# MaciejKozarzewski/AlphaGomoku

Hardware: AMD Instinct MI355X
Metric: MCTS simulations/sec (self-play, 15x15 freestyle) (higher is better)
Workload: dtype f16 (network, fp32 accumulate) + int/fp32 (tree)

## Files before the change

alphagomoku_amd/_lib.py:

```python
import ctypes
import os

_HERE = os.path.dirname(os.path.abspath(__file__))
LIB_PATH = os.environ.get("AGX_LIB_PATH") or os.path.join(_HERE, "libagx.so")


class AgxError(RuntimeError):
    pass


class AgxNetDesc(ctypes.Structure):
    _fields_ = [("rows", ctypes.c_int), ("cols", ctypes.c_int), ("blocks", ctypes.c_int),
                ("filters", ctypes.c_int), ("in_channels", ctypes.c_int), ("value_hidden", ctypes.c_int),
                ("action_values", ctypes.c_int)]


_shared_torch_runtime = None


def share_torch_hip_runtime():
    global _shared_torch_runtime
    if _shared_torch_runtime is not None:
        return _shared_torch_runtime
    import importlib.util
# ... 88 lines not shown
def check(status):
    if status != 0:
        raise AgxError("agx error %d: %s" % (status, lib.agx_last_error().decode()))


class AgxEngineConfig(ctypes.Structure):
    _fields_ = [("rules", ctypes.c_int), ("board_size", ctypes.c_int), ("draw_after", ctypes.c_int), ("n_games", ctypes.c_int),
                ("max_batch_size", ctypes.c_int), ("max_simulations", ctypes.c_int), ("exploration_constant", ctypes.c_float),
                ("exploration_scaling", ctypes.c_float), ("init_to", ctypes.c_int), ("information_leak_threshold", ctypes.c_float),
                ("policy_expansion_threshold", ctypes.c_float), ("tss_max_positions", ctypes.c_int),
                ("tss_table_entries", ctypes.c_uint64), ("zobrist_seed", ctypes.c_uint64), ("node_capacity", ctypes.c_int),
                ("edge_capacity", ctypes.c_int), ("record_capacity", ctypes.c_int), ("record_edge_capacity", ctypes.c_int),
                ("solver_yield_fraction", ctypes.c_float), ("final_selector", ctypes.c_int), ("use_symmetries", ctypes.c_int),
                ("symmetry_seed", ctypes.c_uint64), ("max_children", ctypes.c_int), ("noise_type", ctypes.c_int), ("noise_weight", ctypes.c_float),
                ("noise_seed", ctypes.c_uint64), ("action_values", ctypes.c_int), ("match_mode", ctypes.c_int), ("policy_temperature", ctypes.c_float),
                ("arena_reserve", ctypes.c_float), ("search_threads", ctypes.c_int), ("record_format", ctypes.c_int), ("record_sample_capacity", ctypes.c_int), ("game_end_capacity", ctypes.c_int),
                ("speculative_solver", ctypes.c_int), ("speculative_waves", ctypes.c_int), ("force_expand_root", ctypes.c_int), ("search_buffers", ctypes.c_int)]


class AgxEngineBuffers(ctypes.Structure):
    _fields_ = [("d_nn_features", ctypes.c_void_p), ("d_nn_policy", ctypes.c_void_p), ("d_nn_value", ctypes.c_void_p),
                ("d_nn_action_values", ctypes.c_void_p),
                ("d_nn_list", ctypes.c_void_p), ("d_nn_count", ctypes.c_void_p), ("slots", ctypes.c_int), ("cells", ctypes.c_int)]


class AgxEngineStats(ctypes.Structure):
    _fields_ = [(n, ctypes.c_ulonglong) for n in
                ["evaluated_nodes", "network_evaluations", "information_leaks", "proven_edge_visits", "wasted_expansions",
                 "duplicate_selections", "solver_nodes", "select_levels", "select_edge_reads", "moves_played", "peak_nodes",
                 "peak_edges"]] + [(n, ctypes.c_int) for n in
                                   ["games_finished", "openings_taken", "active_games", "records_used", "record_edges_used",
                                    "first_error", "arena_grows", "arena_releases", "arena_failures", "arena_max_class"]] + \
               [("arena_heap_used", ctypes.c_float), ("speculative_parks", ctypes.c_int), ("speculative_solves", ctypes.c_ulonglong),
                ("speculative_reruns", ctypes.c_ulonglong), ("speculative_deferrals", ctypes.c_ulonglong)]


class AgxEdgeView(ctypes.Structure):
    _fields_ = [("prior", ctypes.c_float), ("win", ctypes.c_float), ("draw", ctypes.c_float), ("visits", ctypes.c_int32),
                ("move", ctypes.c_uint16), ("score", ctypes.c_uint16), ("flag_and_virtual_loss", ctypes.c_uint16),
                ("reserved", ctypes.c_uint16)]


class AgxNodeView(ctypes.Structure):
    _fields_ = [("found", ctypes.c_int), ("visits", ctypes.c_int), ("win", ctypes.c_float), ("draw", ctypes.c_float), ("moves_left", ctypes.c_float)] + \
               [(n, ctypes.c_int) for n in ["score", "flags", "sign_to_move", "depth", "virtual_loss", "n_edges"]]


class AgxGameInfo(ctypes.Structure):
    _fields_ = [(n, ctypes.c_int) for n in ["active", "sign_to_move", "n_moves", "outcome", "error", "opening_id", "games_done",
                                            "n_nodes", "n_edges", "root_visits"]] + \
               [("root_win", ctypes.c_float), ("root_draw", ctypes.c_float), ("root_score", ctypes.c_int), ("root_edges", ctypes.c_int),
                ("grow_pending", ctypes.c_int), ("arena_class", ctypes.c_int), ("root_moves_left", ctypes.c_float), ("max_depth", ctypes.c_int)]


class AgxMoveRecord(ctypes.Structure):
    _fields_ = [("game_serial", ctypes.c_int), ("move_number", ctypes.c_int), ("move", ctypes.c_uint16), ("root_score", ctypes.c_uint16),
                ("root_visits", ctypes.c_int), ("root_win", ctypes.c_float), ("root_draw", ctypes.c_float), ("n_edges", ctypes.c_int),
                ("edge_offset", ctypes.c_int), ("root_flags", ctypes.c_int), ("game_slot", ctypes.c_int), ("game_index", ctypes.c_int),
                ("sample_offset", ctypes.c_int), ("sample_bytes", ctypes.c_int), ("outcome", ctypes.c_int)]


class AgxGameEnd(ctypes.Structure):
    _fields_ = [("game_serial", ctypes.c_int), ("game_slot", ctypes.c_int), ("game_index", ctypes.c_int), ("outcome", ctypes.c_int),
                ("n_moves", ctypes.c_int), ("moves", ctypes.c_uint16 * 400)]


class AgxSavedGame(ctypes.Structure):
# ... 146 lines not shown
```

alphagomoku_amd/csrc/dev_solver.hpp:

```cpp
#ifndef AGX_DEV_SOLVER_HPP_
#define AGX_DEV_SOLVER_HPP_

#include <hip/hip_runtime.h>
#include "engine_types.hpp"

namespace agx
{
	namespace dev
	{
		typedef uint64_t u64;

		__device__ __forceinline__ void wave_sync()
		{
			__builtin_amdgcn_wave_barrier();
			__builtin_amdgcn_fence(__ATOMIC_ACQ_REL, "wavefront");
			__builtin_amdgcn_wave_barrier();
		}

#define AGX_DPP_STEP(V, OP, CTRL, ROWS) V = OP(V, static_cast<uint32_t>(__builtin_amdgcn_update_dpp(0, static_cast<int>(V), CTRL, ROWS, 0xf, false)))
#define AGX_OP_MAX(a, b) max(a, b)
#define AGX_OP_ADD(a, b) ((a) + (b))
#define AGX_OP_XOR(a, b) ((a) ^ (b))
#define AGX_OP_OR(a, b) ((a) | (b))
#define AGX_WAVE_REDUCE(V, OP) do { AGX_DPP_STEP(V, OP, 0x111, 0xf); AGX_DPP_STEP(V, OP, 0x112, 0xf); AGX_DPP_STEP(V, OP, 0x114, 0xf); \
// ... 108 lines not shown
		{
			win = 0.0f;
			draw = 0.0f;
			switch (s_pv(d))
			{
				case 1: draw = 1.0f; break;
				case 2: win = (1000 + s_eval(d)) / 2000.0f; break;
				case 3: win = s_infinite(d) ? 0.0f : 1.0f; break;
				default: break;
			}
		}

		struct alignas(16) Frame
		{
				int base;
				uint16_t size, i;
				uint16_t alpha, beta, original_alpha, best_score;
				uint16_t best_move, move, baseline;
				int16_t depth_remaining;
				uint8_t must_defend, has_initiative, fully_expanded, pad;
				uint32_t ov_slot;
		};
		static_assert(sizeof(Frame) == 32, "frame layout");
		enum Cmd : int { CMD_NONE = 0, CMD_ADD = 1, CMD_UNDO = 2, CMD_DONE = 3 };
#ifndef AGX_LUT_LDS
#define AGX_LUT_LDS 0
#endif
#ifndef AGX_PLACE_OPAQUE_LANE
#define AGX_PLACE_OPAQUE_LANE 1
#endif
		constexpr int NODE_TIME_OVER = 0x40000000;
		constexpr int NODE_COUNT_MASK = NODE_TIME_OVER - 1;
		constexpr int LDS_FRAMES = 42;
		constexpr int OV_CAP = 256;

		template<int N>
		struct SolverSharedT
		{
				static constexpr int DIM = N, HW = N * N;
				static constexpr int CAP2 = (N <= 15) ? 64 : 96, CAP = 24;
				static constexpr int LIST_ITEMS = CAP2 + 7 * CAP;
				static constexpr int SELECT_KEY_BYTES = 3 * (1 + HW) * 8;
#ifndef AGX_ACT_LDS_20
#define AGX_ACT_LDS_20 336
#endif
				static constexpr int ACT_LDS = (N <= 15) ? 448 : AGX_ACT_LDS_20;
				static constexpr int FRAMES = (N <= 15) ? 30 : 34;
				__device__ static constexpr int list_cap(int t) { return (t == 2) ? CAP2 : CAP; }
				__device__ static constexpr int list_off(int t) { return (t == 2) ? 0 : CAP2 + (t - 3) * CAP; }

				u64 lines[6 * N];
				uint32_t act[ACT_LDS];
				Frame frames[FRAMES];
				uint8_t ptype[HW][8];
#if AGX_LUT_LDS
				uint8_t threat_lut[4096];
#endif
				uint8_t threat[HW][2];
				uint16_t items[2][LIST_ITEMS];
				uint16_t pos[2][HW];
				alignas(4) uint16_t count[2][10];
				uint32_t legal[N];
				uint32_t added[N];
				uint32_t row_mask[N];
				uint16_t tmp_list[HW];
				uint16_t foul_cell[64];
				uint8_t foul_flag[64];
				uint8_t board[(HW + 7) / 8 * 8];
				int foul_count;
				int fstack[16][5];
				u64 pf_bucket[8];
				u64 pf_lo;
				int pf_valid;
				uint32_t ov_keys[OV_CAP];
				uint32_t ov_dirty[OV_CAP / 32];
				u64 *ov_data;
				int ov_on, ov_count, ov_overflow, pf_slot;
#ifdef AGX_SOLVER_PROFILE
				unsigned long long prof[8];
				unsigned long long dprof[24];
#endif
				alignas(16) u64 hash_lo;
				u64 hash_hi;
				int phase, level, node_counter, stack_offset;
				int stack_max, error, pending_value, cmd_move;
				u64 time_deadline;
				uint16_t *spill_lists;
				alignas(16) u64 *snap;
				int sign_to_move, depth;
				Frame *spill_frames;
				int cmd, result_score;
		};
		typedef SolverSharedT<MAXN> SolverShared;
#if !defined(AGX_SOLVER_PROFILE)
		static_assert(sizeof(SolverSharedT<15>) <= 10240, "15x15 solver state: sixteen waves per compute unit (160 KB of LDS)");
#endif

		template<class SH>
		__device__ __forceinline__ uint32_t list_get(const SH &sh, int s, int t, int i)
		{
			if (__builtin_expect(i < SH::list_cap(t), 1))
				return sh.items[s][SH::list_off(t) + i];
			uint32_t v;
			asm volatile("global_load_ushort %0, %1, off\n\ts_waitcnt vmcnt(0)" : "=v"(v) : "v"(sh.spill_lists + (s * 10 + t) * SH::HW + i) : "memory");
			return v;
		}
		template<class SH>
		__device__ __forceinline__ void list_set(SH &sh, int s, int t, int i, uint32_t cell)
		{
			if (__builtin_expect(i < SH::list_cap(t), 1))
// ... 1584 lines not shown
						if (distance_to_draw >= 3)
							add_list(opp, 4, s_unknown(4), false);
						mark_neighborhood();
						create_remaining_moves(sh.row_mask, s_unknown(0));
					}
					AGX_PROF_MARK(sh, 7);
					if (fouls_possible_for(own))
						mark_forbidden_moves();
					AGX_PROF_MARK(sh, 9);
					f.fully_expanded = (f.must_defend || mode >= 2) ? 1 : 0;
					return result;
				}
		};

		template<class SH>
		__device__ __forceinline__ int ov_find(const SH &sh, uint32_t bucket, int lane)
		{
			const int cnt = sh.ov_count;
			lane = fresh_lane(lane);
			for (int base = 0; base < cnt; base += 64)
			{
				const u64 m = __ballot(base + lane < cnt && sh.ov_keys[base + lane] == bucket);
				if (m != 0)
					return base + __ffsll(static_cast<long long>(m)) - 1;
			}
			return -1;
		}
		template<class SH>
		__device__ __forceinline__ int ov_create(SH &sh, uint32_t bucket, u64 word, int lane)
		{
			const int p = sh.ov_count;
			if (p >= OV_CAP)
			{
				sh.ov_overflow = 1;
				return -1;
			}
			if (lane < 16)
				global_view(sh.ov_data)[p * 16 + lane] = word;
			if (lane == 0)
			{
				sh.ov_keys[p] = bucket;
				sh.ov_count = p + 1;
			}
			wave_sync();
			return p;
		}

		__device__ __forceinline__ u64 tt_pack(int bound, int depth, uint32_t score, uint32_t move)
		{
			return static_cast<u64>(bound) | (static_cast<u64>(depth) << 8) | (static_cast<u64>(score) << 16) | (static_cast<u64>(move) << 32);
		}
		__device__ __forceinline__ u64 tt_seek(const u64 *tt, u64 bucket_mask, u64 lo, u64 hi)
		{
			const u64 *bucket = tt + 8 * (lo & bucket_mask);
			const u64 KEY = 0xFFFF000000000000ull;
			for (int i = 0; i < 4; i++)
				if (bucket[2 * i] == hi && (bucket[2 * i + 1] & KEY) == (lo & KEY))
					return bucket[2 * i + 1];
			return tt_pack(0, 0, s_unknown(0), 0);
		}
		__device__ __forceinline__ void tt_insert(u64 *tt, u64 bucket_mask, u64 lo, u64 hi, u64 value, int generation)
		{
			const u64 KEY = 0xFFFF000000000000ull;
			value &= ~(KEY | 0xFCull);
			value |= static_cast<u64>(generation) << 2;
			value |= (lo & KEY);
			u64 *bucket = tt + 8 * (lo & bucket_mask);
			const uint32_t score = static_cast<uint32_t>((value >> 16) & 65535u);
			if (s_proven(score) || (value & 3ull) == 3ull)
				for (int i = 0; i < 4; i++)
					if (bucket[2 * i] == hi && (bucket[2 * i + 1] & KEY) == (lo & KEY))
					{
						bucket[2 * i] = hi;
						bucket[2 * i + 1] = value;
						return;
					}
			int idx = 0, best_worth = 0;
			for (int i = 0; i < 4; i++)
// ... 3 lines not shown
				if (i == 0 || worth < best_worth)
				{
					best_worth = worth;
					idx = i;
				}
			}
			bucket[2 * idx] = hi;
			bucket[2 * idx + 1] = value;
		}

#ifndef AGX_TT_LANES
#define AGX_TT_LANES 1
#endif
		__device__ __forceinline__ u64 wave_read64(u64 v, int src_lane)
		{
			const int l = __builtin_amdgcn_readfirstlane(src_lane);
			const uint32_t lo = static_cast<uint32_t>(__builtin_amdgcn_readlane(static_cast<int>(static_cast<uint32_t>(v)), l));
			const uint32_t hi = static_cast<uint32_t>(__builtin_amdgcn_readlane(static_cast<int>(static_cast<uint32_t>(v >> 32)), l));
			return static_cast<u64>(lo) | (static_cast<u64>(hi) << 32);
		}
		__device__ __forceinline__ int tt_match_lanes(u64 word, u64 lo, u64 hi, int lane)
		{
			const u64 KEY = 0xFFFF000000000000ull;
			const bool mine = (lane < 8) && (((lane & 1) == 0) ? (word == hi) : ((word & KEY) == (lo & KEY)));
			const uint32_t m = static_cast<uint32_t>(__ballot(mine));
			const uint32_t both = m & (m >> 1) & 0x55u;
			return (both != 0u) ? ((__ffs(static_cast<int>(both)) - 1) >> 1) : -1;
		}
		__device__ __forceinline__ u64 tt_seek_lanes(u64 word, u64 lo, u64 hi, int lane)
		{
			const int k = tt_match_lanes(word, lo, hi, lane);
			return (k >= 0) ? wave_read64(word, 2 * k + 1) : tt_pack(0, 0, s_unknown(0), 0);
		}
		__device__ __forceinline__ void tt_insert_lanes(u64 *bucket, u64 lo, u64 hi, u64 value, int generation, int lane)
		{
			const u64 KEY = 0xFFFF000000000000ull;
			value &= ~(KEY | 0xFCull);
			value |= static_cast<u64>(generation) << 2;
			value |= (lo & KEY);
			u64 word = 0;
			if (lane < 8)
				word = global_view(bucket)[lane];
			const uint32_t score = static_cast<uint32_t>((value >> 16) & 65535u);
			int idx = -1;
			if (s_proven(score) || (value & 3ull) == 3ull)
				idx = tt_match_lanes(word, lo, hi, lane);
			if (idx < 0)
			{
				const int worth = static_cast<int>((word >> 8) & 255) - (generation - static_cast<int>((word >> 2) & 63));
				const int w0 = __builtin_amdgcn_readlane(worth, 1), w1 = __builtin_amdgcn_readlane(worth, 3), w2 = __builtin_amdgcn_readlane(worth, 5),
						w3 = __builtin_amdgcn_readlane(worth, 7);
				idx = 0;
				int best = w0;
				if (w1 < best) { best = w1; idx = 1; }
				if (w2 < best) { best = w2; idx = 2; }
				if (w3 < best) { best = w3; idx = 3; }
			}
			if (lane < 2)
				global_view(bucket)[2 * idx + lane] = (lane == 0) ? hi : value;
		}

		template<class SH>
		__device__ __forceinline__ uint32_t solver_evaluate(const SH &sh)
		{
			const int lane = static_cast<int>(threadIdx.x);
			const int own = sh.sign_to_move - 1;
			int product = 0;
			if (lane < 20)
			{
				const int side = (lane >= 10) ? 1 : 0, t = lane - 10 * side;
				constexpr u64 OWN_WEIGHTS = 19ull | (49ull << 8) | (76ull << 16) | (170ull << 24) | (33ull << 32) | (159ull << 40) | (252ull << 48);
				constexpr u64 OPP_WEIGHTS = 1ull | (50ull << 9) | (45ull << 18) | (135ull << 27) | (14ull << 36) | (154ull << 45) | (496ull << 54);
				const bool mine = (side == own), weighs = (t >= 2 && t <= 8);
				const int field = weighs ? t - 2 : 0;
				const int magnitude = static_cast<int>(((mine ? OWN_WEIGHTS : OPP_WEIGHTS) >> ((mine ? 8 : 9) * field)) & (mine ? 255ull : 511ull));
				const int weight = weighs ? (mine ? magnitude : -magnitude) : 0;
				product = weight * static_cast<int>(sh.count[side][t]);
			}
			const int result = 12 + static_cast<int>(wave_reduce_add(static_cast<uint32_t>(product)));
			return s_unknown(max(-1000, min(1000, result)));
		}

		template<bool RENJU, class SH>
		__device__ __forceinline__ int solver_run(SH &sh, const EngineDev &E, uint32_t *act, u64 *tt, int generation, int lane, u64 &pf_word,
				uint8_t &pf_pattern, int &pf_pattern_tag, u64 &pf_snap)
		{
			AGX_PROF_BEGIN();
			const u64 zseed = E.zobrist_seed;
			const int n = E.n;
			int phase = sh.phase, level = sh.level;
// ... 12 lines not shown
				sh.error = error;
				sh.hash_lo = hash_lo;
				sh.hash_hi = hash_hi;
				sh.pending_value = static_cast<int>(value);
				sh.cmd_move = move;
				return cmd;
			};
			uint32_t cur_action = 0;
			while (true)
			{
				bool returning = false;
				AGX_PROF_COUNT(sh, 21, 1);
#ifdef AGX_SOLVER_PROFILE
				agx_pt_ = clock64();
				const unsigned long long p0 = wall_clock64();
				unsigned long long p1 = p0, p2 = p0;
#endif
				if (phase == 0)
				{
					f.best_move = 0;
					u64 entry;
					const bool have_pf = sh.pf_valid && sh.pf_lo == hash_lo;
					if (have_pf || sh.ov_on)
					{
						if (sh.ov_on)
						{
							const uint32_t bucket = static_cast<uint32_t>(hash_lo & E.tt_bucket_mask);
							int slot = have_pf ? sh.pf_slot : ov_find(sh, bucket, lane);
							if (!have_pf && lane < 16)
								pf_word = (slot >= 0) ? global_view(sh.ov_data)[slot * 16 + 8 + (lane & 7)] : global_view(tt)[8 * static_cast<u64>(bucket) + (lane & 7)];
							if (slot < 0)
								slot = ov_create(sh, bucket, pf_word, lane);
							f.ov_slot = static_cast<uint32_t>(slot);
						}
#if AGX_TT_LANES
						entry = tt_seek_lanes(pf_word, hash_lo, hash_hi, lane);
					}
					else
					{
						u64 word = 0;
						if (lane < 8)
							word = tt[8 * (hash_lo & E.tt_bucket_mask) + lane];
						entry = tt_seek_lanes(word, hash_lo, hash_hi, lane);
					}
#else
						if (lane < 8)
							sh.pf_bucket[lane] = pf_word;
						wave_sync();
						const u64 KEY = 0xFFFF000000000000ull;
						entry = tt_pack(0, 0, s_unknown(0), 0);
						for (int k = 3; k >= 0; k--)
							if (sh.pf_bucket[2 * k] == hash_hi && (sh.pf_bucket[2 * k + 1] & KEY) == (hash_lo & KEY))
								entry = sh.pf_bucket[2 * k + 1];
					}
					else
						entry = tt_seek(tt, E.tt_bucket_mask, hash_lo, hash_hi);
#endif
					sh.pf_valid = 0;
					bool early = false;
					if (sh.ov_on && sh.ov_overflow)
					{
						error = ERR_OVERLAY;
						value = s_unknown(0);
						early = true;
					}
					else if ((entry & 3ull) != 0ull)
					{
						f.best_move = static_cast<uint16_t>((entry >> 32) & 65535u);
						if (level != 0)
						{
							const uint32_t tt_s = static_cast<uint32_t>((entry >> 16) & 65535u);
							const int b = static_cast<int>(entry & 3ull);
							if (s_proven(tt_s))
							{
								value = tt_s;
								early = true;
							}
							else if (static_cast<int>((entry >> 8) & 255) >= f.depth_remaining && (b == 3 || (b == 1 && tt_s >= f.beta) || (b == 2 && tt_s <= f.alpha)))
							{
								value = tt_s;
								early = true;
							}
						}
					}
#ifdef AGX_SOLVER_PROFILE
					p1 = wall_clock64();
					sh.prof[0] += p1 - p0;
#endif
					if (!early)
					{
						node_counter++;
						if (E.solve_time_ticks != 0ull && wall_clock64() >= sh.time_deadline)
							node_counter |= NODE_TIME_OVER;
// ... 181 lines not shown
						continue;
					}
				}
#ifdef AGX_SOLVER_PROFILE
				const unsigned long long p4 = wall_clock64();
				sh.prof[2] += p4 - p3;
#endif
				if (!returning && phase == 4)
				{
					uint32_t best = f.best_score;
					if (f.size == 0 || (s_loss(best) && !f.fully_expanded))
						best = solver_evaluate(sh);
					if (level > 0)
					{
						const uint32_t umv = frame_get(sh, level - 1).move;
#if AGX_SNAPSHOT_UNDO && AGX_SNAPSHOT_PREFETCH
						pf_snap = *global_view(snap_address<SH>(sh.snap, sh.depth - 1, lane));
						pf_pattern_tag = static_cast<int>(umv);
#elif !AGX_SNAPSHOT_UNDO
						pf_pattern = pattern_prefetch(sh, E, n, umv, false, lane);
						pf_pattern_tag = static_cast<int>(umv);
#endif
					}
					int bound;
					if (best <= f.original_alpha)
						bound = 2;
					else
						bound = (best >= f.beta) ? 1 : 3;
					if (sh.ov_on)
					{
						if (error != ERR_OVERLAY)
						{
							const int slot = static_cast<int>(f.ov_slot);
#if AGX_TT_LANES
							tt_insert_lanes(sh.ov_data + slot * 16 + 8, hash_lo, hash_hi, tt_pack(bound, f.depth_remaining, best, f.best_move), generation, lane);
#else
							tt_insert(sh.ov_data + slot * 16 + 8, 0ull, hash_lo, hash_hi, tt_pack(bound, f.depth_remaining, best, f.best_move), generation);
#endif
							if (lane == 0)
								sh.ov_dirty[slot >> 5] |= 1u << (slot & 31);
						}
					}
					else
#if AGX_TT_LANES
						tt_insert_lanes(tt + 8 * (hash_lo & E.tt_bucket_mask), hash_lo, hash_hi, tt_pack(bound, f.depth_remaining, best, f.best_move), generation, lane);
#else
						tt_insert(tt, E.tt_bucket_mask, hash_lo, hash_hi, tt_pack(bound, f.depth_remaining, best, f.best_move), generation);
#endif
					value = best;
					returning = true;
#ifdef AGX_SOLVER_PROFILE
					sh.prof[3] += wall_clock64() - p4;
#endif
				}
				if (returning)
				{
					if (level == 0)
					{
						sh.frames[0] = f;
						sh.result_score = static_cast<int>(value);
						return yield(CMD_DONE, 0);
					}
					stack_offset -= f.size;
					level--;
					phase = 1;
					return yield(CMD_UNDO, frame_get(sh, level).move);
// ... 8 lines not shown
```

alphagomoku_amd/csrc/engine.hip:

```cpp
#include "agx_internal.hpp"
#include "engine_types.hpp"
#include "dev_mcts.hpp"
#include "tables_host.hpp"
#include "renju_static.hpp"
#include "root_noise.hpp"
#include "sample_v201.hpp"

#include <vector>
#include <thread>
#include <chrono>
#include <mutex>
#include <cstring>
#include <algorithm>

using namespace agx;
using namespace agx::dev;

namespace
{
	__device__ __forceinline__ void select_batch(EngineDev &E, int tg, int g, int lane, uint8_t *sh_board, u64 *sh_cboard, const u64 *sh_keys)
	{
		GameState &gs = E.games[tg];
		GameState &ls = E.games[g];
		DNode *nodes = nodes_of(E, tg, gs.arena);
// ... 289 lines not shown
		u64 *tt = E.tt + static_cast<size_t>(g % E.tt_mod) * (E.tt_bucket_mask + 1ull) * 8ull;
		const int parked_in = (park != nullptr) ? __builtin_amdgcn_readfirstlane(E.park_slot[slot]) : 0;
		int depth_first = 0, stack_before_first = 0;
		if (parked_in != 0)
		{
			static_assert(sizeof(SH) % 8 == 0 && sizeof(SH) / 8 <= SPEC_PARK_WORDS - 8, "park buffer holds the solver's LDS state");
			const u64 *src = E.park_lds + static_cast<size_t>(parked_in - 1) * SPEC_PARK_WORDS;
			u64 *lds = reinterpret_cast<u64*>(&sh);
			for (int i = fresh_lane(lane); i < static_cast<int>(sizeof(SH) / 8); i += 64)
				lds[i] = global_view(src)[i];
			depth_first = static_cast<int>(src[SPEC_PARK_WORDS - 8]);
			stack_before_first = static_cast<int>(src[SPEC_PARK_WORDS - 7]);
			wave_sync();
			park_copy_tails(sh, E, E.park_area0 + parked_in - 1, area, lane);
			if (lane == 0)
			{
				park_point_tails_at(sh, E, area);
				sh.pf_valid = 0;
				E.park_slot[slot] = 0;
			}
			__threadfence();
			wave_sync();
			if (lane == 0)
				__hip_atomic_store(&E.park_owner[parked_in - 1], 0, __ATOMIC_RELEASE, __HIP_MEMORY_SCOPE_AGENT);
		}
		else
		{
		if (lane == 0)
		{
			park_point_tails_at(sh, E, area);
			sh.ov_on = (overlay != nullptr) ? 1 : 0;
			sh.ov_data = overlay;
			sh.ov_count = 0;
			sh.ov_overflow = 0;
			sh.pf_slot = -1;
		}
		if (lane < OV_CAP / 32)
			sh.ov_dirty[lane] = 0;
		}
#ifdef AGX_SOLVER_PROFILE
		unsigned long long c0 = wall_clock64(), c_run = 0, c_place = 0, n_place = 0;
		unsigned long long c1 = c0, t_forbidden = 0;
#endif
		if (parked_in == 0)
		{
		solver_set_board(sh, E, t.board, t.sign_to_move, lane);
		solver_encode_features(sh, E, E.nn_features + static_cast<size_t>(slot) * E.hw, lane);
		#ifdef AGX_SOLVER_PROFILE
		const unsigned long long c_enc = wall_clock64();
		#endif
		if (RENJU)
			solver_encode_forbidden(sh, E, E.nn_features + static_cast<size_t>(slot) * E.hw, lane);
		#ifdef AGX_SOLVER_PROFILE
		c1 = wall_clock64();
		t_forbidden = c1 - c_enc;
		#endif
		u64 lo = 0, hi = 0;
		for (int i = lane; i < E.hw; i += 64)
		{
			const int v = sh.board[i];
			if (v == 1 || v == 2)
			{
				lo ^= zobrist_word(E.zobrist_seed, 2 * (2 * i + v - 1));
				hi ^= zobrist_word(E.zobrist_seed, 2 * (2 * i + v - 1) + 1);
			}
		}
		lo = wave_reduce_xor64(lo);
// ... 301 lines not shown
			{
				gs.solve_pos = k;
				gs.solve_pending = 1;
				gs.stats[5] += solver_nodes;
			}
			return;
		}
		const unsigned long long scheduled = idle ? 0ull : schedule_to_nn(sh, E, g, gs, n_tasks, lane);
		if (lane == 0)
		{
			if (!idle)
			{
				gs.solve_pos = 0;
				gs.solve_pending = 0;
				gs.stats[5] += solver_nodes;
				gs.stats[1] += scheduled;
			}
			atomicAdd(&E.counters[E.yield_counter], 1);
		}
	}


	template<class SH>
	__device__ __forceinline__ void spec_flush(const SH &sh, SpecTask &h, int nodes, uint32_t flags0, float moves_left0, int lane)
	{
		const int cnt = sh.ov_count;
		for (int i = lane; i < cnt; i += 64)
			h.keys[i] = sh.ov_keys[i];
		if (lane < OV_CAP / 32)
			h.dirty[lane] = sh.ov_dirty[lane];
		if (lane == 0)
		{
			h.count = cnt;
			h.overflow = (sh.ov_overflow || sh.error == ERR_OVERLAY) ? 1 : 0;
			h.nodes = nodes;
			h.flags0 = flags0;
			h.moves_left0 = moves_left0;
			h.solved = 1;
		}
	}
#ifndef AGX_DEFER_ON_EMPTY_QUEUE
#define AGX_DEFER_ON_EMPTY_QUEUE 0
#endif
	struct SpecCommit
	{
		int game, k, first;
			bool table_changed;
			unsigned long long nodes, solved, reruns;
	};
	template<class SH>
	__device__ __forceinline__ int spec_commit_game(SH &sh, const EngineDev &E, SpecCommit &c, int lane, const int *c_done, int defer_threshold, const int *c_queue, int count)
	{
		const int g = c.game;
		GameState &gs = E.games[g];
		const int n_tasks = gs.n_tasks;
		u64 *tt = E.tt + static_cast<size_t>(g % E.tt_mod) * (E.tt_bucket_mask + 1ull) * 8ull;
		for (int k = c.k; k < n_tasks; k++)
		{
			const int slot = g * E.batch + k;
			SpecTask &h = E.spec_tasks[slot];
			if (h.solved == 0)
				continue;
			DTask &t = E.tasks[slot];
			const u64 *ov = E.spec_overlay + static_cast<size_t>(slot) * (SPEC_OV_CAP * 16);
			const int cnt = h.count;
			bool valid = (h.overflow == 0);
			{
				bool bad = (cnt < 0 || cnt > SPEC_OV_CAP);
				for (int i = lane; !bad && i < cnt; i += 64)
					bad = static_cast<u64>(h.keys[i]) > E.tt_bucket_mask;
				if (__ballot(bad) != 0ull)
				{
					if (lane == 0)
					{
						gs.error = ERR_SPEC_STATE;
						h.solved = 0;
					}
					continue;
				}
			}
			if (valid && c.table_changed)
			{
				bool mismatch = false;
				for (int base = 0; base < cnt; base += 8)
				{
					const int p = base + (lane >> 3), w = lane & 7;
					if (p < cnt)
						mismatch = mismatch || (ov[p * 16 + w] != tt[8 * static_cast<u64>(h.keys[p]) + w]);
				}
				valid = (__ballot(mismatch) == 0ull);
			}
			if (!valid)
			{
				int done = 0;
				if (lane == 0)
					done = __hip_atomic_load(c_done, __ATOMIC_RELAXED, __HIP_MEMORY_SCOPE_AGENT);
#if AGX_DEFER_ON_EMPTY_QUEUE
				int dry = 0;
				if (lane == 0 && defer_threshold != 0x7FFFFFFF)
					dry = (__hip_atomic_load(c_queue + 3, __ATOMIC_RELAXED, __HIP_MEMORY_SCOPE_AGENT) >= count
							&& __hip_atomic_load(c_queue + 1, __ATOMIC_RELAXED, __HIP_MEMORY_SCOPE_AGENT) >= __hip_atomic_load(c_queue + 2, __ATOMIC_RELAXED, __HIP_MEMORY_SCOPE_AGENT)) ? 1 : 0;
				const bool defer = (__builtin_amdgcn_readfirstlane(done) >= defer_threshold || __builtin_amdgcn_readfirstlane(dry) != 0) && k > c.first;
#else
				const bool defer = __builtin_amdgcn_readfirstlane(done) >= defer_threshold && k > c.first;
#endif
				for (int j = k; j < (defer ? n_tasks : k + 1); j++)
				{
					SpecTask &hj = E.spec_tasks[g * E.batch + j];
					if (hj.solved != 0 && lane == 0)
					{
						DTask &tj = E.tasks[g * E.batch + j];
						tj.flags = hj.flags0;
						tj.win = 0.0f;
						tj.draw = 0.0f;
						tj.moves_left = hj.moves_left0;
						hj.solved = 0;
					}
				}
				wave_sync();
				if (defer)
				{
					if (lane == 0)
					{
						gs.solve_pos = k;
						gs.solve_pending = 1;
						gs.stats[5] += c.nodes;
						gs.spec_stats[0] += c.solved;
						gs.spec_stats[1] += c.reruns;
						gs.spec_stats[2] += 1;
					}
					return -2;
				}
				c.solved++;
				c.reruns++;
				c.table_changed = true;
				c.k = k + 1;
				return k;
			}
			bool any = false;
			for (int base = 0; base < cnt; base += 8)
			{
				const int p = base + (lane >> 3), w = lane & 7;
				if (p < cnt && ((h.dirty[p >> 5] >> (p & 31)) & 1u))
				{
					tt[8 * static_cast<u64>(h.keys[p]) + w] = ov[p * 16 + 8 + w];
					any = true;
				}
			}
			c.table_changed = c.table_changed || (__ballot(any) != 0ull);
			c.nodes += static_cast<unsigned long long>(h.nodes);
			c.solved++;
			if (lane == 0)
				h.solved = 0;
			wave_sync();
		}
		const unsigned long long scheduled = schedule_to_nn(sh, E, g, gs, n_tasks, lane);
		if (lane == 0)
		{
			gs.solve_pos = 0;
			gs.solve_pending = 0;
			gs.stats[5] += c.nodes;
			gs.stats[1] += scheduled;
			gs.spec_stats[0] += c.solved;
			gs.spec_stats[1] += c.reruns;
#ifdef AGX_SPEC_PROFILE
			E.spec_trace[4 * g + 3] = c.reruns * 16 + c.solved;
#endif
		}
		return -1;
	}

#ifdef AGX_SPEC_PROFILE
#define SPEC_T(var) unsigned long long var = wall_clock64()
#define SPEC_ADD(k, v) do { if (lane == 0) atomicAdd(&E.spec_prof[k], static_cast<unsigned long long>(v)); } while (0)
#define SPEC_MAX(k, v) do { if (lane == 0) atomicMax(&E.spec_prof[k], static_cast<unsigned long long>(v)); } while (0)
#define SPEC_WAVE_EXIT() do { if (lane == 0) { unsigned long long *w_ = E.spec_trace + 4 * (static_cast<size_t>(E.n_games) + E.spec_group * E.spec_waves + blockIdx.x); \
		w_[0] = t_selected; w_[1] = wall_clock64(); w_[2] = wave_solves; w_[3] = wave_waited; } } while (0)
#else
#define SPEC_T(var) do { } while (0)
#define SPEC_ADD(k, v) do { } while (0)
#define SPEC_MAX(k, v) do { } while (0)
#define SPEC_WAVE_EXIT() do { } while (0)
#endif
#ifndef AGX_SPEC_WAVES
#define AGX_SPEC_WAVES 3
#endif
#ifndef AGX_SPEC_WAVES_15
#define AGX_SPEC_WAVES_15 4
#endif
	constexpr int spec_waves_per_simd(int nfix) { return (nfix == 15) ? AGX_SPEC_WAVES_15 : AGX_SPEC_WAVES; }
	template<bool RENJU, int NFIX>
	__global__ __launch_bounds__(64, spec_waves_per_simd(NFIX)) void k_search_spec(EngineDev E, int count)
	{
		if (NFIX != 0)
		{
			E.n = NFIX;
			E.hw = NFIX * NFIX;
// ... 213 lines not shown
			SPEC_T(t_s0);
			const bool parked = solve_task<RENJU>(sh, E, g, t, slot, E.games[g].generation, lane, n1, area,
					speculative ? E.spec_overlay + static_cast<size_t>(slot) * (SPEC_OV_CAP * 16) : nullptr, (SPEC_PARKS && speculative) ? &park_ctl : nullptr);
			if (!speculative)
			{
				commit.nodes += n1;
				continue;
			}
			if (parked)
			{
				SPEC_T(t_parked);
				SPEC_ADD(3, t_parked - t_s0);
				continue;
			}
			spec_flush(sh, E.spec_tasks[slot], static_cast<int>(n1), flags0, moves_left0, lane);
			SPEC_T(t_solved);
			SPEC_ADD(3, t_solved - t_s0);
			SPEC_ADD(6, 1);
#ifdef AGX_SPEC_PROFILE
			wave_solves++;
#endif
			__threadfence();
			int left = 0;
			if (lane == 0)
				left = __hip_atomic_fetch_add(&E.spec_left[g], -1, __ATOMIC_ACQ_REL, __HIP_MEMORY_SCOPE_AGENT);
			left = __builtin_amdgcn_readfirstlane(left);
			if (left == 1)
			{
				__threadfence();
				commit.game = g;
				commit.k = 0;
				commit.first = E.games[g].solve_pending ? E.games[g].solve_pos : 0;
				commit.table_changed = false;
				commit.nodes = commit.solved = commit.reruns = 0;
				__builtin_amdgcn_s_setprio(3);
#ifdef AGX_SPEC_PROFILE
				t_commit0 = wall_clock64();
#endif
			}
		}
	}

#ifndef AGX_WIDE_BACKUP
#define AGX_WIDE_BACKUP 1
#endif
	__global__ __launch_bounds__(64) void k_expand(EngineDev E)
	{
		__shared__ float e_prior[MAXHW], e_win[MAXHW], e_draw[MAXHW];
		__shared__ uint16_t e_move[MAXHW], e_score[MAXHW];
		__shared__ float sh_sum;
		__shared__ u64 sort_keys[512];
		const int g0 = E.g0 + blockIdx.x, lane = threadIdx.x;
		const int tg = E.shared_tree ? 0 : g0;
		GameState &gs = E.games[tg];
		if (!gs.active || gs.error != 0 || gs.outcome != 0 || (!E.shared_tree && gs.solve_pending) || gs.grow_pending == 1 || gs.grow_pending == 3)
			return;
		use_game_arenas(E, tg);
		DNode *nodes = nodes_of(E, tg, gs.arena);
		DEdge *edges = edges_of(E, tg, gs.arena);
		int *ht = ht_of(E, tg);
		const int n = E.n, hw = E.hw;
		const int first_lane = E.shared_tree ? E.grp_first : g0, last_lane = E.shared_tree ? E.grp_first + E.grp_count - 1 : g0;
		if (E.shared_tree && gs.grow_pending != 0 && gs.grow_owner != E.grp_first)
			return;
		{
			int need_edges = gs.n_edges, need_nodes = gs.n_nodes;
			for (int lg = first_lane; lg <= last_lane; lg++)
// ... 2162 lines not shown
	d.park_fraction = parking ? SPEC_PARK_FRACTION : 0.0f;
	if (const char *pf = std::getenv("AGX_PARK_FRACTION"))
		if (parking && std::atof(pf) > 0.0)
			d.park_fraction = std::min(1.0f, static_cast<float>(std::atof(pf)));
	AGX_TRY(dev_alloc(e, &d.park_slot, G * d.batch));
	AGX_TRY(dev_alloc(e, &d.park_owner, SPEC_PARK_POOL));
	AGX_TRY(dev_alloc(e, &d.parts_done, 2 * G));
	if (!e->sizing_only)
		(void) hipMemset(d.parts_done, 0, 2 * G * sizeof(int));
	AGX_TRY(dev_alloc(e, &d.park_lds, parking ? static_cast<size_t>(SPEC_PARK_POOL) * SPEC_PARK_WORDS : 1));
	if (!e->sizing_only)
		(void) hipMemset(d.park_slot, 0, G * d.batch * sizeof(int));
	if (!e->sizing_only)
		(void) hipMemset(d.park_owner, 0, SPEC_PARK_POOL * sizeof(int));
	AGX_TRY(dev_alloc(e, &d.act, areas * d.act_cap));
	AGX_TRY(dev_alloc(e, &d.list_spill, areas * 20 * static_cast<size_t>(MAXHW)));
	AGX_TRY(dev_alloc(e, &d.frame_spill, areas * MAX_FRAMES));
	AGX_TRY(dev_alloc(e, &d.snap_spill, areas * static_cast<size_t>(d.hw + 2) * 64));
	d.spec_group = 0;
	d.spec_waves = e->spec_waves;
	AGX_TRY(dev_alloc(e, &d.spec_watchdog, 16));
	if (!e->sizing_only)
		(void) hipMemset(d.spec_watchdog, 0, 16 * sizeof(int));
	AGX_TRY(dev_alloc(e, &d.spec_prof, 16));
	AGX_TRY(dev_alloc(e, &d.spec_trace, 4 * (G + static_cast<size_t>(std::max(e->spec_waves, 16)))));
	if (!e->sizing_only)
		(void) hipMemset(d.spec_trace, 0, 4 * (G + static_cast<size_t>(std::max(e->spec_waves, 16))) * sizeof(unsigned long long));
	if (!e->sizing_only)
		(void) hipMemset(d.spec_prof, 0, 16 * sizeof(unsigned long long));
	AGX_TRY(dev_alloc(e, &d.spec_items, e->speculative ? G * d.batch + 16 * static_cast<size_t>(SPEC_QUEUE_SLACK) : 1));
	AGX_TRY(dev_alloc(e, &d.spec_left, e->speculative ? G : 1));
	AGX_TRY(dev_alloc(e, &d.spec_tasks, e->speculative ? G * d.batch : 1));
	AGX_TRY(dev_alloc(e, &d.spec_overlay, e->speculative ? G * d.batch * (SPEC_OV_CAP * 16) : 1));
	AGX_TRY(dev_alloc(e, &d.tt, G * buckets * 8));
	AGX_TRY(dev_upload(e, &d.t_pattern, tables.pattern));
	AGX_TRY(dev_upload(e, &d.t_ho3, tables.half_open_three));
	AGX_TRY(dev_upload(e, &d.t_threat, tables.threat));
	{
		std::vector<uint8_t> packed(4096);
		for (int i = 0; i < 4096; i++)
			packed[i] = static_cast<uint8_t>((tables.threat[2 * i] & 15u) | ((tables.threat[2 * i + 1] & 15u) << 4));
		AGX_TRY(dev_upload(e, &d.t_threat_packed, packed));
	}
	AGX_TRY(dev_upload(e, &d.t_defense, tables.defense));
	AGX_TRY(dev_upload(e, &d.nc_keys, nc_keys));
	AGX_TRY(dev_upload(e, &d.zob, e->zobrist));
	AGX_TRY(dev_alloc(e, &d.nn_features, G * d.batch * d.hw));
	AGX_TRY(dev_alloc(e, &d.nn_policy, G * d.batch * d.hw));
	AGX_TRY(dev_alloc(e, &d.nn_value, G * d.batch * 3));
	d.has_q = cfg->action_values ? 1 : 0;
	d.match_mode = cfg->match_mode ? 1 : 0;
	d.prune_root = (cfg->match_mode || !cfg->force_expand_root) ? 1 : 0;
	d.search_buffers = (cfg->search_buffers == 2) ? 2 : 1;
	d.shared_tree = (cfg->search_threads > 1 || d.search_buffers == 2) ? 1 : 0;
	d.tt_mod = (d.search_buffers == 2) ? std::max(1, cfg->search_threads) : static_cast<int>(G);
	d.grp_first = 0;
	d.grp_count = static_cast<int>(G);
	d.policy_temperature = cfg->policy_temperature;
	AGX_TRY(dev_alloc(e, &d.nn_q, d.has_q ? G * d.batch * d.hw * 2 : 1));
	AGX_TRY(dev_alloc(e, &d.noise, d.noise_type ? G * d.hw : 1));
	AGX_TRY(dev_alloc(e, &d.nn_list, G * d.batch));
	AGX_TRY(dev_alloc(e, &d.counters, N_COUNTERS));
	AGX_TRY(dev_alloc(e, &d.records, static_cast<size_t>(d.record_cap)));
	AGX_TRY(dev_alloc(e, &d.record_edges, (d.record_format & 1) ? static_cast<size_t>(d.record_edge_cap) : 1));
	AGX_TRY(dev_alloc(e, &d.samples, (d.record_format & 2) ? static_cast<size_t>(d.sample_cap) : 4));
	AGX_TRY(dev_alloc(e, &d.game_ends, static_cast<size_t>(d.game_end_cap)));
// ... 822 lines not shown
	*waves = e->speculative ? e->spec_waves : 0;
	return AGX_OK;
}
int agx_engine_device_bytes(AgxEngine *e, unsigned long long *bytes)
{
	AGX_REQUIRE(e != nullptr && bytes != nullptr, AGX_ERR_INVALID, "agx_engine_device_bytes: null argument");
	*bytes = e->device_bytes;
	return AGX_OK;
}
int agx_engine_stats(AgxEngine *e, AgxEngineStats *out)
{
	AGX_REQUIRE(e != nullptr && out != nullptr, AGX_ERR_INVALID, "agx_engine_stats: null argument");
	std::vector<GameState> games(e->dev.n_games);
	AGX_HIP_CHECK(hipMemcpy(games.data(), e->dev.games, games.size() * sizeof(GameState), hipMemcpyDeviceToHost));
	int counters[16];
	AGX_HIP_CHECK(hipMemcpy(counters, e->dev.counters, sizeof(counters), hipMemcpyDeviceToHost));
	std::memset(out, 0, sizeof(*out));
	for (const GameState &g : games)
	{
		out->evaluated_nodes += g.stats[0];
		out->network_evaluations += g.stats[1];
		out->information_leaks += g.stats[2];
		out->proven_edge_visits += g.stats[3];
		out->wasted_expansions += g.stats[4];
		out->solver_nodes += g.stats[5];
		out->select_levels += g.stats[6];
		out->select_edge_reads += g.stats[7];
		out->moves_played += g.stats[8];
		out->duplicate_selections += g.stats[9];
		out->speculative_solves += g.spec_stats[0];
		out->speculative_reruns += g.spec_stats[1];
		out->speculative_deferrals += g.spec_stats[2];
		out->speculative_parks += static_cast<int>(g.spec_stats[3]);
		out->peak_nodes = std::max<unsigned long long>(out->peak_nodes, g.stats[10]);
		out->peak_edges = std::max<unsigned long long>(out->peak_edges, g.stats[11]);
		out->active_games += g.active ? 1 : 0;
		if (g.error != 0 && out->first_error == 0)
			out->first_error = g.error;
	}
	if (e->speculative)
	{
		int w[16];
		AGX_HIP_CHECK(hipMemcpy(w, e->dev.spec_watchdog, sizeof(w), hipMemcpyDeviceToHost));
		if (w[0] != 0)
			fprintf(stderr, "[k_search_spec watchdog] a wave waited in vain for queue slot %d: head %d, tail %d, games selected %d of %d, select cursor %d\n", w[1], w[2], w[3], w[4],
					w[5], w[6]);
	}
#ifdef AGX_SPEC_PROFILE
	if (getenv("AGX_SPEC_TRACE"))
	{
		std::vector<unsigned long long> tr(4 * games.size());
		AGX_HIP_CHECK(hipMemcpy(tr.data(), e->dev.spec_trace, tr.size() * sizeof(unsigned long long), hipMemcpyDeviceToHost));
		FILE *f = fopen(getenv("AGX_SPEC_TRACE"), "w");
		if (f != nullptr)
		{
			for (size_t g = 0; g < games.size(); g++)
				fprintf(f, "%llu %llu %llu %llu\n", tr[4 * g], tr[4 * g + 1], tr[4 * g + 2], tr[4 * g + 3]);
			fclose(f);
		}
		std::vector<unsigned long long> wv(4 * static_cast<size_t>(std::max(e->spec_waves, 16)));
		AGX_HIP_CHECK(hipMemcpy(wv.data(), e->dev.spec_trace + 4 * games.size(), wv.size() * sizeof(unsigned long long), hipMemcpyDeviceToHost));
		f = fopen((std::string(getenv("AGX_SPEC_TRACE")) + ".waves").c_str(), "w");
		if (f != nullptr)
		{
			for (size_t w = 0; 4 * w < wv.size(); w++)
				fprintf(f, "%llu %llu %llu %llu\n", wv[4 * w], wv[4 * w + 1], wv[4 * w + 2], wv[4 * w + 3]);
// ... 629 lines not shown
```

alphagomoku_amd/csrc/engine_types.hpp:

```cpp
#ifndef AGX_ENGINE_TYPES_HPP_
#define AGX_ENGINE_TYPES_HPP_

#include <cstdint>

namespace agx
{
	constexpr int MAXN = 20;
	constexpr int MAXHW = MAXN * MAXN;
	constexpr int BWORDS = 13;
	constexpr int PATH_CAP = 256;
	constexpr int SPEC_PARK_POOL = 128;
	constexpr int SPEC_PARK_WORDS = 2048 + 8;
	constexpr int MAX_FRAMES = 104;
	constexpr int OPENING_CAP = 32;

	struct alignas(16) FrameBytes { uint32_t w[8]; };

	struct DEdge
	{
			float prior;
			float win;
			float draw;
			int32_t visits;
			uint16_t move;
// ... 53 lines not shown
	struct GameState
	{
			int32_t active;
			int32_t sign_to_move;
			int32_t n_moves;
			int32_t outcome;
			int32_t root;
			int32_t n_nodes;
			int32_t n_edges;
			int32_t arena;
			int32_t n_tasks;
			int32_t need_move;
			int32_t generation;
			int32_t error;
			int32_t opening_id;
			int32_t games_done;
			int32_t solve_pos;
			int32_t solve_pending;
			int32_t nn_queued;
			int32_t noise_ready;
			int32_t my_sign;
			int32_t restart_id;
			int32_t match_score[4];
			int32_t arena_class;
			int32_t grow_pending;
			int32_t node_cap, edge_cap, ht_cap, grow_count;
			int32_t grow_owner, max_depth;
			uint64_t node_off[2], edge_off[2], ht_off;
			uint64_t new_node_off[2], new_edge_off[2], new_ht_off;
			uint64_t root_hash;
			uint64_t cboard[BWORDS];
			unsigned long long prof[8];
			unsigned long long dprof[24];
			unsigned long long spec_stats[4];
			unsigned long long stats[12];
			uint8_t board[MAXHW];
			uint16_t moves[MAXHW];
	};

	struct MoveRecordHeader
	{
			int32_t game_serial;
			int32_t move_number;
			uint16_t move;
			uint16_t root_score;
			int32_t root_visits;
			float root_win;
			float root_draw;
			int32_t n_edges;
			int32_t edge_offset;
			int32_t root_flags;
			int32_t game_slot;
			int32_t game_index;
			int32_t sample_offset;
			int32_t sample_bytes;
			int32_t outcome;
	};
	struct GameEndRecord
	{
			int32_t game_serial, game_slot, game_index;
			int32_t outcome;
			int32_t n_moves;
			uint16_t moves[MAXHW];
	};

	constexpr int SPEC_OV_CAP = 256;
	constexpr int SPEC_COUNTER0 = 64;
	constexpr int SPEC_QUEUE_SLACK = 8192;
	constexpr int N_COUNTERS = 192;
	struct SpecTask
	{
			int32_t solved;
			int32_t count;
			int32_t overflow;
			int32_t nodes;
			uint32_t flags0;
			float moves_left0;
			uint32_t pad[2];
			uint32_t dirty[SPEC_OV_CAP / 32];
			uint32_t keys[SPEC_OV_CAP];
	};

	constexpr int ARENA_CLASSES = 6;

	struct ArenaBundle
	{
			uint64_t node_off[2], edge_off[2], ht_off;
	};
	struct ArenaHeap
	{
			uint64_t node_cursor, edge_cursor, ht_cursor;
			uint64_t node_total, edge_total, ht_total;
			int32_t free_count[ARENA_CLASSES];
			int32_t free_capacity;
			int32_t grows, releases, failures, lock;
	};

	enum EngineError : int32_t
	{
		ERR_NONE = 0, ERR_NODE_CAPACITY = 1, ERR_EDGE_CAPACITY = 2, ERR_PATH_CAPACITY = 3, ERR_ACTION_STACK = 4, ERR_HASH_TABLE = 5, ERR_RECORDS = 6, ERR_FRAMES = 7, ERR_SPEC_STATE = 8,
		ERR_OVERLAY = 100
	};

	struct EngineDev
	{
			int rules, n, hw, draw_after;
			int n_games, batch, max_sims;
			int batch_limit;
			float c_puct, c_scale;
			int init_to;
			float leak_threshold, expansion_threshold;
// ... 31 lines not shown
			FrameBytes *frame_spill;
			uint64_t *snap_spill;
			uint64_t *tt;
			const uint8_t *t_pattern;
			const uint8_t *t_ho3;
			const uint8_t *t_threat;
			const uint8_t *t_threat_packed;
			const uint16_t *t_defense;
			const uint64_t *nc_keys;
			const uint64_t *zob;
			const uint16_t *openings;
			uint32_t *nn_features;
			float *nn_policy;
			float *nn_value;
			float *nn_q;
			int has_q;
			int match_merged;
			int prune_root;
			int match_mode;
			int shared_tree;
			int search_buffers;
			int tt_mod;
			int grp_first, grp_count;
			int spec_on;
			int spec_group;
			int *spec_watchdog;
			unsigned long long *spec_trace;
			unsigned long long *spec_prof;
			int spec_waves;
			int *spec_items;
			int *spec_left;
			SpecTask *spec_tasks;
			uint64_t *spec_overlay;
			int *park_slot;
			int *park_owner;
			int *parts_done;
			uint64_t *park_lds;
			int park_area0;
			float park_fraction;
			int *nn_list;
			int *counters;
			MoveRecordHeader *records;
			DEdge *record_edges;
			uint8_t *samples;
			GameEndRecord *game_ends;
	};
}

#endif
```

include/agx.h:

```cpp
#ifndef AGX_H_
#define AGX_H_

#include <stddef.h>
#include <stdint.h>

#ifdef __cplusplus
extern "C" {
#endif

#define AGX_OK 0
#define AGX_ERR_INVALID 1
#define AGX_ERR_HIP 2
#define AGX_ERR_UNSUPPORTED 3
#define AGX_ERR_STATE 4

enum AgxRules { AGX_FREESTYLE = 0, AGX_STANDARD = 1, AGX_RENJU = 2, AGX_CARO5 = 3, AGX_CARO6 = 4 };

enum AgxSign { AGX_NONE = 0, AGX_CROSS = 1, AGX_CIRCLE = 2, AGX_ILLEGAL = 3 };

const char* agx_last_error(void);
int agx_version(void);
const char* agx_build_hash(void);
int agx_set_device(int device);
int agx_device_count(int* count);
// ... 81 lines not shown
	int slots;
	int cells;
} AgxEngineBuffers;

typedef struct AgxEngineStats
{
	unsigned long long evaluated_nodes;
	unsigned long long network_evaluations;
	unsigned long long information_leaks;
	unsigned long long proven_edge_visits;
	unsigned long long wasted_expansions;
	unsigned long long duplicate_selections;
	unsigned long long solver_nodes;
	unsigned long long select_levels;
	unsigned long long select_edge_reads;
	unsigned long long moves_played;
	unsigned long long peak_nodes;
	unsigned long long peak_edges;
	int games_finished;
	int openings_taken;
	int active_games;
	int records_used;
	int record_edges_used;
	int first_error;
	int arena_grows;
	int arena_releases;
	int arena_failures;
	int arena_max_class;
	float arena_heap_used;
	int speculative_parks;
	unsigned long long speculative_solves;
	unsigned long long speculative_reruns;
	unsigned long long speculative_deferrals;
} AgxEngineStats;

typedef struct AgxEdgeView
{
	float prior, win, draw;
	int32_t visits;
	uint16_t move;
	uint16_t score;
	uint16_t flag_and_virtual_loss;
	uint16_t reserved;
} AgxEdgeView;

typedef struct AgxGameInfo
{
	int active, sign_to_move, n_moves, outcome, error, opening_id, games_done, n_nodes, n_edges;
	int root_visits;
	float root_win, root_draw;
	int root_score;
	int root_edges;
	int grow_pending;
	int arena_class;
	float root_moves_left;
	int max_depth;
} AgxGameInfo;

typedef struct AgxMoveRecord
{
	int game_serial, move_number;
	uint16_t move, root_score;
	int root_visits;
	float root_win, root_draw;
	int n_edges, edge_offset;
	int root_flags;
// ... 209 lines not shown
```

Measured before the change: 1.029 million.

## Replay logged overlay TT operations to salvage speculative solves on table change

Speculative solver tasks now record every transposition-table seek and insert on their overlay buckets into a per-task global log. At commit time, if a touched bucket changed since the snapshot, the log is replayed against the current table contents. If every seek would still have returned the same entry, the solve is accepted and the overlay is rewritten, so a full rerun is skipped. This adds global-memory writes for each logged seek and insert, extra log memory, and replay work during commit.

```diff
diff --git a/alphagomoku_amd/_lib.py b/alphagomoku_amd/_lib.py
--- a/alphagomoku_amd/_lib.py
+++ b/alphagomoku_amd/_lib.py
@@ -144,7 +144,8 @@
                                    ["games_finished", "openings_taken", "active_games", "records_used", "record_edges_used",
                                     "first_error", "arena_grows", "arena_releases", "arena_failures", "arena_max_class"]] + \
                [("arena_heap_used", ctypes.c_float), ("speculative_parks", ctypes.c_int), ("speculative_solves", ctypes.c_ulonglong),
-                ("speculative_reruns", ctypes.c_ulonglong), ("speculative_deferrals", ctypes.c_ulonglong)]
+                ("speculative_reruns", ctypes.c_ulonglong), ("speculative_deferrals", ctypes.c_ulonglong),
+                ("speculative_replays", ctypes.c_ulonglong)]
 
 
 class AgxEdgeView(ctypes.Structure):
diff --git a/alphagomoku_amd/csrc/dev_solver.hpp b/alphagomoku_amd/csrc/dev_solver.hpp
--- a/alphagomoku_amd/csrc/dev_solver.hpp
+++ b/alphagomoku_amd/csrc/dev_solver.hpp
@@ -164,6 +164,7 @@
 		constexpr int NODE_TIME_OVER = 0x40000000;
 		constexpr int NODE_COUNT_MASK = NODE_TIME_OVER - 1;
 		constexpr int LDS_FRAMES = 42;
+		constexpr int OV_FULL = 1, OV_LOG_FULL = 2, OV_LOG_SHIFT = 2;
 		constexpr int OV_CAP = 256;
 
 		template<int N>
@@ -207,7 +208,7 @@
 				uint32_t ov_keys[OV_CAP];
 				uint32_t ov_dirty[OV_CAP / 32];
 				u64 *ov_data;
-				int ov_on, ov_count, ov_overflow, pf_slot;
+				int ov_on, ov_count, ov_state, pf_slot;
 #ifdef AGX_SOLVER_PROFILE
 				unsigned long long prof[8];
 				unsigned long long dprof[24];
@@ -1858,7 +1859,7 @@
 			const int p = sh.ov_count;
 			if (p >= OV_CAP)
 			{
-				sh.ov_overflow = 1;
+				sh.ov_state |= OV_FULL;
 				return -1;
 			}
 			if (lane < 16)
@@ -1870,6 +1871,24 @@
 			}
 			wave_sync();
 			return p;
+		}
+		constexpr int OV_LOG_SEEK = 1, OV_LOG_INSERT = 2;
+		template<class SH>
+		__device__ __forceinline__ void ov_log(SH &sh, const EngineDev &E, int kind, int slot, u64 lo, u64 hi, u64 value, int lane)
+		{
+			const int state = sh.ov_state, n = state >> OV_LOG_SHIFT;
+			if (n >= E.spec_log_cap)
+			{
+				sh.ov_state = state | OV_LOG_FULL;
+				return;
+			}
+			const u64 task = static_cast<u64>(sh.ov_data - E.spec_overlay) / (OV_CAP * 16);
+			u64 *rec = E.spec_log + (task * static_cast<u64>(E.spec_log_cap) + static_cast<u64>(n)) * 4;
+			lane = fresh_lane(lane);
+			const u64 w = (lane == 0) ? static_cast<u64>(static_cast<uint32_t>(slot) | (static_cast<uint32_t>(kind) << 16)) : (lane == 1) ? hi : (lane == 2) ? lo : value;
+			if (lane < 4)
+				global_view(rec)[lane] = w;
+			sh.ov_state = state + (1 << OV_LOG_SHIFT);
 		}
 
 		__device__ __forceinline__ u64 tt_pack(int bound, int depth, uint32_t score, uint32_t move)
@@ -1939,15 +1958,12 @@
 			const int k = tt_match_lanes(word, lo, hi, lane);
 			return (k >= 0) ? wave_read64(word, 2 * k + 1) : tt_pack(0, 0, s_unknown(0), 0);
 		}
-		__device__ __forceinline__ void tt_insert_lanes(u64 *bucket, u64 lo, u64 hi, u64 value, int generation, int lane)
+		__device__ __forceinline__ int tt_insert_slot(u64 word, u64 lo, u64 hi, u64 &value, int generation, int lane)
 		{
 			const u64 KEY = 0xFFFF000000000000ull;
 			value &= ~(KEY | 0xFCull);
 			value |= static_cast<u64>(generation) << 2;
 			value |= (lo & KEY);
-			u64 word = 0;
-			if (lane < 8)
-				word = global_view(bucket)[lane];
 			const uint32_t score = static_cast<uint32_t>((value >> 16) & 65535u);
 			int idx = -1;
 			if (s_proven(score) || (value & 3ull) == 3ull)
@@ -1963,6 +1979,14 @@
 				if (w2 < best) { best = w2; idx = 2; }
 				if (w3 < best) { best = w3; idx = 3; }
 			}
+			return idx;
+		}
+		__device__ __forceinline__ void tt_insert_lanes(u64 *bucket, u64 lo, u64 hi, u64 value, int generation, int lane)
+		{
+			u64 word = 0;
+			if (lane < 8)
+				word = global_view(bucket)[lane];
+			const int idx = tt_insert_slot(word, lo, hi, value, generation, lane);
 			if (lane < 2)
 				global_view(bucket)[2 * idx + lane] = (lane == 0) ? hi : value;
 		}
@@ -2041,6 +2065,8 @@
 							if (slot < 0)
 								slot = ov_create(sh, bucket, pf_word, lane);
 							f.ov_slot = static_cast<uint32_t>(slot);
+							if (slot >= 0)
+								ov_log(sh, E, OV_LOG_SEEK, slot, hash_lo, hash_hi, 0ull, lane);
 						}
 #if AGX_TT_LANES
 						entry = tt_seek_lanes(pf_word, hash_lo, hash_hi, lane);
@@ -2067,7 +2093,7 @@
 #endif
 					sh.pf_valid = 0;
 					bool early = false;
-					if (sh.ov_on && sh.ov_overflow)
+					if (sh.ov_on && (sh.ov_state & OV_FULL))
 					{
 						error = ERR_OVERLAY;
 						value = s_unknown(0);
@@ -2315,6 +2341,7 @@
 						if (error != ERR_OVERLAY)
 						{
 							const int slot = static_cast<int>(f.ov_slot);
+							ov_log(sh, E, OV_LOG_INSERT, slot, hash_lo, hash_hi, tt_pack(bound, f.depth_remaining, best, f.best_move), lane);
 #if AGX_TT_LANES
 							tt_insert_lanes(sh.ov_data + slot * 16 + 8, hash_lo, hash_hi, tt_pack(bound, f.depth_remaining, best, f.best_move), generation, lane);
 #else
diff --git a/alphagomoku_amd/csrc/engine.hip b/alphagomoku_amd/csrc/engine.hip
--- a/alphagomoku_amd/csrc/engine.hip
+++ b/alphagomoku_amd/csrc/engine.hip
@@ -345,7 +345,7 @@
 			sh.ov_on = (overlay != nullptr) ? 1 : 0;
 			sh.ov_data = overlay;
 			sh.ov_count = 0;
-			sh.ov_overflow = 0;
+			sh.ov_state = 0;
 			sh.pf_slot = -1;
 		}
 		if (lane < OV_CAP / 32)
@@ -713,7 +713,9 @@
 		if (lane == 0)
 		{
 			h.count = cnt;
-			h.overflow = (sh.ov_overflow || sh.error == ERR_OVERLAY) ? 1 : 0;
+			h.overflow = ((sh.ov_state & OV_FULL) || sh.error == ERR_OVERLAY) ? 1 : 0;
+			h.log_count = sh.ov_state >> OV_LOG_SHIFT;
+			h.log_full = (sh.ov_state & OV_LOG_FULL) ? 1 : 0;
 			h.nodes = nodes;
 			h.flags0 = flags0;
 			h.moves_left0 = moves_left0;
@@ -727,8 +729,65 @@
 	{
 		int game, k, first;
 			bool table_changed;
-			unsigned long long nodes, solved, reruns;
+			unsigned long long nodes, solved, reruns, replays;
 	};
+	__device__ __forceinline__ bool spec_replay(const EngineDev &E, const SpecTask &h, u64 *ov, const u64 *tt, int slot, int generation, int lane)
+	{
+		const int cnt = h.count, n_log = h.log_count;
+		if (h.log_full != 0 || n_log < 0 || n_log > E.spec_log_cap)
+			return false;
+		const u64 *log = E.spec_log + static_cast<size_t>(slot) * static_cast<size_t>(E.spec_log_cap) * 4;
+		for (int base = 0; base < cnt; base += 8)
+		{
+			const int p = base + (lane >> 3), w = lane & 7;
+			u64 changed = __ballot(p < cnt && ov[p * 16 + w] != tt[8 * static_cast<u64>(h.keys[min(p, cnt - 1)]) + w]);
+			while (changed != 0ull)
+			{
+				const int q8 = (__ffsll(static_cast<long long>(changed)) - 1) >> 3, q = base + q8;
+				changed &= ~(0xFFull << (8 * q8));
+				u64 first = 0, now = 0;
+				if (lane < 8)
+				{
+					first = ov[q * 16 + lane];
+					now = tt[8 * static_cast<u64>(h.keys[q]) + lane];
+				}
+				for (int r0 = 0; r0 < n_log; r0 += 64)
+				{
+					const int r = r0 + lane;
+					u64 mine = __ballot(r < n_log && static_cast<int>(log[4 * static_cast<size_t>(min(r, n_log - 1))] & 0xFFFFull) == q);
+					while (mine != 0ull)
+					{
+						const u64 *rec = log + 4 * static_cast<size_t>(r0 + __ffsll(static_cast<long long>(mine)) - 1);
+						mine &= mine - 1ull;
+						const int kind = static_cast<int>((rec[0] >> 16) & 0xFFFFull);
+						const u64 hi = rec[1], lo = rec[2];
+						if (kind == OV_LOG_SEEK)
+						{
+							if (tt_seek_lanes(first, lo, hi, lane) != tt_seek_lanes(now, lo, hi, lane))
+								return false;
+						}
+						else if (kind == OV_LOG_INSERT)
+						{
+							u64 v_first = rec[3], v_now = rec[3];
+							const int i_first = tt_insert_slot(first, lo, hi, v_first, generation, lane);
+							const int i_now = tt_insert_slot(now, lo, hi, v_now, generation, lane);
+							if ((lane >> 1) == i_first)
+								first = (lane & 1) ? v_first : hi;
+							if ((lane >> 1) == i_now)
+								now = (lane & 1) ? v_now : hi;
+						}
+						else
+							return false;
+					}
+				}
+				if (lane < 8)
+					ov[q * 16 + 8 + lane] = now;
+			}
+		}
+		__threadfence();
+		wave_sync();
+		return true;
+	}
 	template<class SH>
 	__device__ __forceinline__ int spec_commit_game(SH &sh, const EngineDev &E, SpecCommit &c, int lane, const int *c_done, int defer_threshold, const int *c_queue, int count)
 	{
@@ -743,8 +802,9 @@
 			if (h.solved == 0)
 				continue;
 			DTask &t = E.tasks[slot];
-			const u64 *ov = E.spec_overlay + static_cast<size_t>(slot) * (SPEC_OV_CAP * 16);
+			u64 *ov = E.spec_overlay + static_cast<size_t>(slot) * (SPEC_OV_CAP * 16);
 			const int cnt = h.count;
+			bool replayed = false;
 			bool valid = (h.overflow == 0);
 			{
 				bool bad = (cnt < 0 || cnt > SPEC_OV_CAP);
@@ -770,6 +830,11 @@
 						mismatch = mismatch || (ov[p * 16 + w] != tt[8 * static_cast<u64>(h.keys[p]) + w]);
 				}
 				valid = (__ballot(mismatch) == 0ull);
+				if (!valid)
+				{
+					valid = spec_replay(E, h, ov, tt, slot, gs.generation, lane);
+					replayed = valid;
+				}
 			}
 			if (!valid)
 			{
@@ -809,6 +874,7 @@
 						gs.spec_stats[0] += c.solved;
 						gs.spec_stats[1] += c.reruns;
 						gs.spec_stats[2] += 1;
+						gs.spec_stats[4] += c.replays;
 					}
 					return -2;
 				}
@@ -831,6 +897,8 @@
 			c.table_changed = c.table_changed || (__ballot(any) != 0ull);
 			c.nodes += static_cast<unsigned long long>(h.nodes);
 			c.solved++;
+			if (replayed)
+				c.replays++;
 			if (lane == 0)
 				h.solved = 0;
 			wave_sync();
@@ -844,6 +912,7 @@
 			gs.stats[1] += scheduled;
 			gs.spec_stats[0] += c.solved;
 			gs.spec_stats[1] += c.reruns;
+			gs.spec_stats[4] += c.replays;
 #ifdef AGX_SPEC_PROFILE
 			E.spec_trace[4 * g + 3] = c.reruns * 16 + c.solved;
 #endif
@@ -1123,7 +1192,7 @@
 				commit.k = 0;
 				commit.first = E.games[g].solve_pending ? E.games[g].solve_pos : 0;
 				commit.table_changed = false;
-				commit.nodes = commit.solved = commit.reruns = 0;
+				commit.nodes = commit.solved = commit.reruns = commit.replays = 0;
 				__builtin_amdgcn_s_setprio(3);
 #ifdef AGX_SPEC_PROFILE
 				t_commit0 = wall_clock64();
@@ -3352,6 +3421,10 @@
 	AGX_TRY(dev_alloc(e, &d.spec_left, e->speculative ? G : 1));
 	AGX_TRY(dev_alloc(e, &d.spec_tasks, e->speculative ? G * d.batch : 1));
 	AGX_TRY(dev_alloc(e, &d.spec_overlay, e->speculative ? G * d.batch * (SPEC_OV_CAP * 16) : 1));
+	d.spec_log_cap = SPEC_LOG_CAP;
+	if (const char *cap = std::getenv("AGX_SPEC_LOG_CAP"))
+		d.spec_log_cap = std::max(1, std::min(std::atoi(cap), SPEC_LOG_CAP));
+	AGX_TRY(dev_alloc(e, &d.spec_log, e->speculative ? G * d.batch * static_cast<size_t>(d.spec_log_cap) * 4 : 1));
 	AGX_TRY(dev_alloc(e, &d.tt, G * buckets * 8));
 	AGX_TRY(dev_upload(e, &d.t_pattern, tables.pattern));
 	AGX_TRY(dev_upload(e, &d.t_ho3, tables.half_open_three));
@@ -4240,6 +4313,7 @@
 		out->speculative_reruns += g.spec_stats[1];
 		out->speculative_deferrals += g.spec_stats[2];
 		out->speculative_parks += static_cast<int>(g.spec_stats[3]);
+		out->speculative_replays += g.spec_stats[4];
 		out->peak_nodes = std::max<unsigned long long>(out->peak_nodes, g.stats[10]);
 		out->peak_edges = std::max<unsigned long long>(out->peak_edges, g.stats[11]);
 		out->active_games += g.active ? 1 : 0;
diff --git a/alphagomoku_amd/csrc/engine_types.hpp b/alphagomoku_amd/csrc/engine_types.hpp
--- a/alphagomoku_amd/csrc/engine_types.hpp
+++ b/alphagomoku_amd/csrc/engine_types.hpp
@@ -109,7 +109,7 @@
 			uint64_t cboard[BWORDS];
 			unsigned long long prof[8];
 			unsigned long long dprof[24];
-			unsigned long long spec_stats[4];
+			unsigned long long spec_stats[5];
 			unsigned long long stats[12];
 			uint8_t board[MAXHW];
 			uint16_t moves[MAXHW];
@@ -142,6 +142,7 @@
 	};
 
 	constexpr int SPEC_OV_CAP = 256;
+	constexpr int SPEC_LOG_CAP = 1024;
 	constexpr int SPEC_COUNTER0 = 64;
 	constexpr int SPEC_QUEUE_SLACK = 8192;
 	constexpr int N_COUNTERS = 192;
@@ -153,7 +154,8 @@
 			int32_t nodes;
 			uint32_t flags0;
 			float moves_left0;
-			uint32_t pad[2];
+			int32_t log_count;
+			int32_t log_full;
 			uint32_t dirty[SPEC_OV_CAP / 32];
 			uint32_t keys[SPEC_OV_CAP];
 	};
@@ -251,6 +253,8 @@
 			int *spec_left;
 			SpecTask *spec_tasks;
 			uint64_t *spec_overlay;
+			uint64_t *spec_log;
+			int spec_log_cap;
 			int *park_slot;
 			int *park_owner;
 			int *parts_done;
diff --git a/include/agx.h b/include/agx.h
--- a/include/agx.h
+++ b/include/agx.h
@@ -137,6 +137,7 @@
 	unsigned long long speculative_solves;
 	unsigned long long speculative_reruns;
 	unsigned long long speculative_deferrals;
+	unsigned long long speculative_replays;
 } AgxEngineStats;
 
 typedef struct AgxEdgeView
```

Result: slower. 982,700 (-4.5%).
